# amazon-science/instruct-video-to-video

Measured on AMD Instinct MI355X. Metric: denoised video-frames/sec (16f@256x384, 50 DDIM steps), higher is better.
Workload: dtype fp16; 1 GPU; C2: 1 clip/step = VAE-encode + 50 DDIM steps (3-way CFG, text 7.5 / video 1.5) + VAE-decode, 16 frames @ 256x384, random-init full-width UNet+VAE; 5 independent clips in flight per GPU (stacked into every UNet launch, B = 3 x clips); frames=16, height=256, width=384, ddim_steps=50, clips_per_gpu=5, parallelism=clip-parallel x1, one all_gather, hip_graph=True, cfg_branch_streams=False, concurrent_clips=5, clip_mode=stacked, driver_mode=False, full=False

## Files before the change

### instruct-video-to-video_amd/csrc/attention.hip

```cpp
#include "common.h"
#include "gemm_dma.h"
#include <cstdlib>
#include <algorithm>

typedef unsigned int uint4v __attribute__((ext_vector_type(4)));

__device__ __forceinline__ unsigned pack2h(float a, float b) {
    auto h = __builtin_amdgcn_cvt_pkrtz(a, b);
    return __builtin_bit_cast(unsigned, h);
}

typedef float float2v __attribute__((ext_vector_type(2)));
typedef _Float16 half2v __attribute__((ext_vector_type(2)));
__device__ __forceinline__ float col_max(float v) {
    float a = v, b = v;
    asm volatile("s_nop 1\n\tv_permlane16_swap_b32 %0, %1\n\ts_nop 1" : "+v"(a), "+v"(b));
    a = b = fmaxf(a, b);
    asm volatile("s_nop 1\n\tv_permlane32_swap_b32 %0, %1\n\ts_nop 1" : "+v"(a), "+v"(b));
    return fmaxf(a, b);
}
__device__ __forceinline__ float col_sum(float v) {
    float a = v, b = v;
    asm volatile("s_nop 1\n\tv_permlane16_swap_b32 %0, %1\n\ts_nop 1" : "+v"(a), "+v"(b));
    a = b = a + b;
    asm volatile("s_nop 1\n\tv_permlane32_swap_b32 %0, %1\n\ts_nop 1" : "+v"(a), "+v"(b));
    return a + b;
}

#ifndef ATTN_REP_PREFETCH
#define ATTN_REP_PREFETCH 1
#endif
#ifndef ATTN_SINGLE_ST16
#define ATTN_SINGLE_ST16 1
#endif
template <int D, int NW, int KVT, int QB, bool FOLD = false, bool SINGLE = false, bool REP = false>
__global__ __launch_bounds__(NW * 64, (NW == 8 && D == 40) ? 4 : SINGLE ? 3 : (D == 80 && QB == 2) ? 2 : 1) void attn_kernel(insv2v_attention_desc p) {
    constexpr int NBUF = SINGLE ? 1 : 2;
    static_assert(!(SINGLE && FOLD), "the single-tile form is for the unfolded kernel");
    static_assert(!REP || SINGLE, "only the single-tile form keeps its tile across problems");
    constexpr int DP = (D + 31) / 32 * 32;
    constexpr int DTA = (D + 15) / 16;
    static_assert(!FOLD || DP > D, "FOLD needs a zero-padded contraction column");
    constexpr bool ONES = FOLD && (D % 16) != 0;
    constexpr int FKK = D / 32, FG = (D % 32) / 8, FE = D % 8;
    constexpr bool VDMA = FOLD && KVT == 64 && (D % 8) == 0 && (D % 16 == 0 || ONES);
    constexpr bool ST16 = SINGLE && !REP && ATTN_SINGLE_ST16 && (DTA % 2 == 0) && (D % 32 == 0);
    constexpr int NCBF = D / 16;
    constexpr bool VHALF = (D % 16) != 0;
    constexpr int VIMG = NCBF * KVT * 32 + (VHALF ? KVT * 16 : 0);
    constexpr int NPV = VIMG / 1024, NPVW = (NPV + NW - 1) / NW;
    constexpr int VT_LD = KVT + 4;
    constexpr int NKB = KVT / 32;
    constexpr bool KSWZ = DP == 64;
    constexpr int KLD = KSWZ ? DP : DP + 8;
    constexpr int DT = DP / 16;
    constexpr int KS = DP / 32;
    constexpr int NT = NW * 64;
    constexpr int KCH = DP / 8;
    constexpr int K_ITERS = (KVT * KCH + NT - 1) / NT;
    constexpr int VP = KVT / 2;
    constexpr int V_ITERS = (VP * KCH + NT - 1) / NT;
    extern __shared__ __attribute__((aligned(16))) char smem[];
    half_t* sK = (half_t*)smem;
    half_t* sVt = sK + NBUF * KVT * KLD;

    const int tid = threadIdx.x, lane = tid & 63, wid = tid >> 6;
    const int g = lane >> 4, qc = lane & 15;
    const int nqb = (p.seq_q + 16 * NW * QB - 1) / (16 * NW * QB), nhd = p.heads;
    const int lin = xcd_remap(blockIdx.x, gridDim.x);
    const int qblk = lin % nqb, head = (lin / nqb) % nhd;
    const int nrep = REP ? p.kv_inner : 1;
    const int z0 = (lin / (nqb * nhd)) * nrep;
    constexpr int d = D;
    const half_t* K = (const half_t*)p.k + (int64_t)(z0 / p.kv_inner) * p.kv_outer + (int64_t)(z0 % p.kv_inner) * p.kv_step + head * d;
    const half_t* V = (const half_t*)p.v + (int64_t)(z0 / p.kv_inner) * p.kv_outer + (int64_t)(z0 % p.kv_inner) * p.kv_step + head * d;

    int qrow[QB];
    half8 qf[QB][KS];
#pragma unroll
    for (int b = 0; b < QB; ++b) qrow[b] = (qblk * NW + wid) * (16 * QB) + b * 16 + qc;
    auto load_q = [&](int z) {
        const half_t* Q = (const half_t*)p.q + (int64_t)(z / p.q_inner) * p.q_outer + (int64_t)(z % p.q_inner) * p.q_step + head * d;
#pragma unroll
        for (int b = 0; b < QB; ++b) {
#pragma unroll
            for (int kk = 0; kk < KS; ++kk) {
                const int c = kk * 32 + g * 8;
                half8 v = {0, 0, 0, 0, 0, 0, 0, 0};
                if (qrow[b] < p.seq_q && c < d) v = *(const half8*)(Q + (int64_t)qrow[b] * p.q_rs + c);
                if (FOLD) {
                    const float c2q = p.scale * 1.4426950408889634f;
#pragma unroll
                    for (int e = 0; e < 8; ++e) v[e] = (half_t)((float)v[e] * c2q);
                }
                qf[b][kk] = v;
            }
        }
    };
    load_q(z0);
    const unsigned kone = (FOLD && g == FG) ? ((FE & 1) ? 0x3C000000u : 0x00003C00u) : 0u;

    uint4 rk[K_ITERS], rv[V_ITERS][2];
    const srd_t rK = make_srd(K), rVv = make_srd(V);
    constexpr int KROW_B = KLD * 2;
    constexpr bool KDMA = (KVT * KROW_B) % 1024 == 0;
    constexpr int NPK = KVT * KROW_B / 1024, NPKW = (NPK + NW - 1) / NW;
    static_assert(!VDMA || KDMA, "the V DMA path shares the K path's end-of-tile wait");
    int kd_key[KDMA ? NPKW : 1];
    unsigned kd_src[KDMA ? NPKW : 1];
    unsigned kd_off[KDMA ? NPKW : 1] = {};
    if (KDMA) {
#pragma unroll
        for (int i = 0; i < NPKW; ++i) {
            const int o = (wid + NW * i) * 1024 + lane * 16;
            const int key = o / KROW_B, slot = (o - key * KROW_B) >> 4;
            const int ch = KSWZ ? (slot ^ ((key >> 1) & 7)) : slot;
            kd_key[i] = (wid + NW * i < NPK && ch * 8 < d) ? key : (1 << 30);
            kd_src[i] = (unsigned)((key * (int)p.k_rs + ch * 8) * 2);
        }
    }
    int vd_key[VDMA ? NPVW : 1];
    unsigned vd_src[VDMA ? NPVW : 1];
    unsigned vd_off[VDMA ? NPVW : 1] = {};
    char* const sV = (char*)(sK + NBUF * KVT * KLD);
    if (VDMA) {
#pragma unroll
        for (int i = 0; i < NPVW; ++i) {
            const int pc = wid + NW * i;
            const bool full = pc < 2 * NCBF;
            const int key = full ? (pc & 1) * 32 + (lane >> 1) : lane;
            const int ch = full ? (pc >> 1) * 16 + (lane & 1) * 8 : NCBF * 16;
            vd_key[i] = pc < NPV ? key : (1 << 30);
            vd_src[i] = (unsigned)((key * (int)p.v_rs + ch) * 2);
        }
        if (tid < 4) ((unsigned*)(sV + 2 * VIMG))[tid] = tid == 0 ? 0x00003C00u : 0u;
    }
    auto load_vdma = [&](int t, int buf) {
        const int key0 = t * KVT;
#pragma unroll
        for (int i = 0; i < NPVW; ++i) {
            vd_off[i] = key0 + vd_key[i] < p.seq_k ? vd_src[i] : OOB_OFFSET;
            if (wid + NW * i < NPV)
                dma16(rVv, vd_off[i], key0 * (int)p.v_rs * 2, sV + buf * VIMG + (wid + NW * i) * 1024);
        }
    };
    auto load_k = [&](int t, int buf) {
        const int key0 = t * KVT;
        if (KDMA) {
            char* dst = (char*)(sK + buf * KVT * KLD) + wid * 1024;
#pragma unroll
            for (int i = 0; i < NPKW; ++i) {
                kd_off[i] = key0 + kd_key[i] < p.seq_k ? kd_src[i] : OOB_OFFSET;
                if (wid + NW * i < NPK)
                    dma16(rK, kd_off[i], key0 * (int)p.k_rs * 2, dst + i * NW * 1024);
            }
            return;
        }
#pragma unroll
        for (int i = 0; i < K_ITERS; ++i) {
            const int e = tid + NT * i;
            const int key = e / KCH, ch = e - key * KCH;
            const bool ok = e < KVT * KCH && key0 + key < p.seq_k && ch * 8 < d;
            const uint4v v = __builtin_amdgcn_raw_buffer_load_b128(rK, ok ? (unsigned)(((key0 + key) * (int)p.k_rs + ch * 8) * 2) : OOB_OFFSET, 0, 0);
            rk[i] = make_uint4(v[0], v[1], v[2], v[3]);
        }
    };
    auto load_v = [&](int t) {
        const int key0 = t * KVT;
#pragma unroll
        for (int i = 0; i < V_ITERS; ++i) {
            const int e = tid + NT * i;
            const int ch = e / VP, kp = e - ch * VP;
#pragma unroll
            for (int h = 0; h < 2; ++h) {
                const int key = key0 + 2 * kp + h;
                const bool ok = e < VP * KCH && key < p.seq_k && ch * 8 < d;
                const uint4v v = __builtin_amdgcn_raw_buffer_load_b128(rVv, ok ? (unsigned)((key * (int)p.v_rs + ch * 8) * 2) : OOB_OFFSET, 0, 0);
                rv[i][h] = make_uint4(v[0], v[1], v[2], v[3]);
            }
        }
    };
    auto load_tile = [&](int t, int buf) {
        if constexpr (VDMA) load_vdma(t, buf);
        else load_v(t);
        load_k(t, buf);
    };
    auto store_tile = [&](int buf) {
        half_t* k = sK + buf * KVT * KLD;
        half_t* vt = sVt + buf * DP * VT_LD;
#pragma unroll
        for (int i = 0; i < K_ITERS; ++i) {
            const int e = tid + NT * i;
            const int key = e / KCH, ch = e - key * KCH;
            const int pc = KSWZ ? (ch ^ ((key >> 1) & 7)) : ch;
            if (!KDMA && e < KVT * KCH) *(uint4*)(k + key * KLD + pc * 8) = rk[i];
        }
        if constexpr (VDMA) return;
#pragma unroll
        for (int i = 0; i < V_ITERS; ++i) {
            const int e = tid + NT * i;
            const int ch = e / VP, kp = e - ch * VP;
            if (e < VP * KCH) {
                const unsigned short* h0 = (const unsigned short*)&rv[i][0];
                const unsigned short* h1 = (const unsigned short*)&rv[i][1];
#pragma unroll
                for (int j = 0; j < 8; ++j) {
                    unsigned w = (unsigned)h0[j] | ((unsigned)h1[j] << 16);
                    if (ONES && j == D % 8 && ch == D / 8) w = 0x3C003C00u;
                    *(unsigned*)(vt + (ch * 8 + j) * VT_LD + 2 * kp) = w;
                }
            }
        }
    };

    floatx4 acc[QB][DT];
    float m_run[QB], l_run[QB];
    const float c2 = p.scale * 1.4426950408889634f;

    const unsigned sv_lds = (unsigned)(uintptr_t)(__attribute__((address_space(3))) char*)sV;
    const unsigned va_full = sv_lds + (g * 4 + (qc >> 2)) * 32 + (qc & 3) * 8;
    const bool va_const = (qc & 3) >= 2;
    const unsigned va_half0 = va_const ? sv_lds + 2 * VIMG + ((qc & 3) == 3 ? 8 : 0) : sv_lds + NCBF * KVT * 32 + (g * 4 + (qc >> 2)) * 16 + (qc & 3) * 8;
    const unsigned va_hstep_buf = va_const ? 0u : (unsigned)VIMG, va_hstep_kb = va_const ? 0u : 512u, va_hstep_hi = va_const ? 0u : 256u;

    const int ntiles = (p.seq_k + KVT - 1) / KVT;
    load_tile(0, 0);
    store_tile(0);
    if (KDMA) wait_vmcnt<0>();
    __syncthreads();

#pragma unroll 1
  for (int rep = 0; rep < nrep; ++rep) {
    const int z = z0 + rep;
#if !ATTN_REP_PREFETCH
    if (REP && rep > 0) load_q(z);
#endif
    half_t* O = (half_t*)p.o + (int64_t)(z / p.o_inner) * p.o_outer + (int64_t)(z % p.o_inner) * p.o_step + head * d;
#pragma unroll
    for (int b = 0; b < QB; ++b) {
        m_run[b] = FOLD ? 0.f : -1.0e30f;
        l_run[b] = 0.f;
#pragma unroll
        for (int i = 0; i < DT; ++i) acc[b][i] = (floatx4){0.f, 0.f, 0.f, 0.f};
    }
    for (int t = 0; t < ntiles; ++t) {
        const int cur = t & 1;
        const half_t* k = sK + cur * KVT * KLD;
        const half_t* vt = sVt + cur * DP * VT_LD;
        const int key0 = t * KVT;
        const bool ragged = key0 + KVT > p.seq_k;

        floatx4 s[QB][NKB][2];
#pragma unroll
        for (int kb = 0; kb < NKB; ++kb)
#pragma unroll
            for (int sub = 0; sub < 2; ++sub) {
#pragma unroll
                for (int b = 0; b < QB; ++b) s[b][kb][sub] = (floatx4){0.f, 0.f, 0.f, 0.f};
                const half_t* kr = k + (kb * 32 + sub * 16 + qc) * KLD;
                const int ksw = KSWZ ? ((qc >> 1) & 7) : 0;
#pragma unroll
                for (int kk = 0; kk < KS; ++kk) {
                    half8 kf = *(const half8*)(kr + (((kk * 4 + g) ^ ksw) * 8));
                    if (FOLD && kk == FKK) {
                        uint4v ku = __builtin_bit_cast(uint4v, kf);
                        ku[FE / 2] |= kone;
                        kf = __builtin_bit_cast(half8, ku);
                    }
#pragma unroll
                    for (int b = 0; b < QB; ++b)
                        s[b][kb][sub] = __builtin_amdgcn_mfma_f32_16x16x32_f16(kf, qf[b][kk], s[b][kb][sub], 0, 0, 0);
                }
            }
        if (t + 1 < ntiles) load_tile(t + 1, cur ^ 1);
#if ATTN_REP_PREFETCH
        if (REP && rep + 1 < nrep) load_q(z + 1);
#endif
        half8 pf[QB][NKB];
#pragma unroll
        for (int b = 0; b < QB; ++b) {
            if (ragged || p.causal) {
                const int kmax = p.causal ? min(p.seq_k - 1, qrow[b]) : p.seq_k - 1;
                const int rel = kmax - key0 - g * 4;
#pragma unroll
                for (int kb = 0; kb < NKB; ++kb)
#pragma unroll
                    for (int sub = 0; sub < 2; ++sub)
#pragma unroll
                        for (int r = 0; r < 4; ++r)
                            if (kb * 32 + sub * 16 + r > rel) s[b][kb][sub][r] = -1.0e30f;
            }
            if constexpr (FOLD) {
                float mx = s[b][0][0][0];
#pragma unroll
                for (int kb = 0; kb < NKB; ++kb)
#pragma unroll
                    for (int sub = 0; sub < 2; ++sub)
#pragma unroll
                        for (int r = 0; r < 4; ++r) mx = fmaxf(mx, s[b][kb][sub][r]);
                if (t == 0 || __builtin_amdgcn_ballot_w64(mx > 8.f) != 0) {
                    mx = col_max(mx);
                    const float want = m_run[b] + (t == 0 ? mx : fmaxf(mx, 0.f));
                    const float mnew = (float)(half_t)want;
                    const float shift = mnew - m_run[b];
                    m_run[b] = mnew;
                    if (t > 0) {
                        const float alpha = __builtin_amdgcn_exp2f(-shift);
                        if (!ONES) l_run[b] *= alpha;
#pragma unroll
                        for (int i = 0; i < DTA; ++i)
#pragma unroll
                            for (int r = 0; r < 4; ++r) acc[b][i][r] *= alpha;
                    }
#pragma unroll
                    for (int kb = 0; kb < NKB; ++kb)
#pragma unroll
                        for (int sub = 0; sub < 2; ++sub)
#pragma unroll
                            for (int r = 0; r < 4; ++r) s[b][kb][sub][r] -= shift;
                    if (g == FG) qf[b][FKK][FE] = (half_t)(-mnew);
                }
                const half2v ones = {(_Float16)1.f, (_Float16)1.f};
                float psum = 0.f;
#pragma unroll
                for (int kb = 0; kb < NKB; ++kb) {
                    uint4v pk;
#pragma unroll
                    for (int sub = 0; sub < 2; ++sub)
#pragma unroll
                        for (int h = 0; h < 2; ++h) {
                            const unsigned u = pack2h(__builtin_amdgcn_exp2f(s[b][kb][sub][2 * h]), __builtin_amdgcn_exp2f(s[b][kb][sub][2 * h + 1]));
                            if (!ONES) psum = __builtin_amdgcn_fdot2(__builtin_bit_cast(half2v, u), ones, psum, false);
                            pk[sub * 2 + h] = u;
                        }
                    pf[b][kb] = __builtin_bit_cast(half8, pk);
                }
                if (!ONES) l_run[b] += psum;
                continue;
            }
            float mx = m_run[b];
#pragma unroll
            for (int kb = 0; kb < NKB; ++kb)
#pragma unroll
                for (int sub = 0; sub < 2; ++sub)
#pragma unroll
                    for (int r = 0; r < 4; ++r) mx = fmaxf(mx, s[b][kb][sub][r]);
            mx = col_max(mx);
            if (__builtin_amdgcn_ballot_w64(mx > m_run[b]) != 0) {
                const float alpha = __builtin_amdgcn_exp2f((m_run[b] - mx) * c2);
                m_run[b] = mx;
                l_run[b] *= alpha;
#pragma unroll
                for (int i = 0; i < DTA; ++i)
#pragma unroll
                    for (int r = 0; r < 4; ++r) acc[b][i][r] *= alpha;
            }
            const float2v c2v = {c2, c2}, mcv = {-mx * c2, -mx * c2};
            const half2v ones = {(_Float16)1.f, (_Float16)1.f};
            float psum = 0.f;
#pragma unroll
            for (int kb = 0; kb < NKB; ++kb) {
                uint4v pk;
#pragma unroll
                for (int sub = 0; sub < 2; ++sub)
#pragma unroll
                    for (int h = 0; h < 2; ++h) {
                        float2v x = {s[b][kb][sub][2 * h], s[b][kb][sub][2 * h + 1]};
                        x = __builtin_elementwise_fma(x, c2v, mcv);
                        const unsigned u = pack2h(__builtin_amdgcn_exp2f(x[0]), __builtin_amdgcn_exp2f(x[1]));
                        psum = __builtin_amdgcn_fdot2(__builtin_bit_cast(half2v, u), ones, psum, false);
                        pk[sub * 2 + h] = u;
                    }
                pf[b][kb] = __builtin_bit_cast(half8, pk);
            }
            l_run[b] += psum;
        }

#pragma unroll
        for (int kb = 0; kb < NKB; ++kb) {
#pragma unroll
            for (int i = 0; i < DTA; ++i) {
                half4 lo, hi;
                if constexpr (VDMA) {
                    typedef __fp16 fp16x4 __attribute__((__vector_size__(4 * sizeof(__fp16))));
                    typedef __attribute__((address_space(3))) fp16x4* lds4_t;
                    if (i < NCBF) {
                        const unsigned a = va_full + cur * VIMG + i * (KVT * 32) + kb * 1024;
                        lo = __builtin_bit_cast(half4, __builtin_amdgcn_ds_read_tr16_b64_v4f16((lds4_t)(uintptr_t)a));
                        hi = __builtin_bit_cast(half4, __builtin_amdgcn_ds_read_tr16_b64_v4f16((lds4_t)(uintptr_t)(a + 512)));
                    } else {
                        const unsigned a = va_half0 + cur * va_hstep_buf + kb * va_hstep_kb;
                        lo = __builtin_bit_cast(half4, __builtin_amdgcn_ds_read_tr16_b64_v4f16((lds4_t)(uintptr_t)a));
                        hi = __builtin_bit_cast(half4, __builtin_amdgcn_ds_read_tr16_b64_v4f16((lds4_t)(uintptr_t)(a + va_hstep_hi)));
                    }
                } else {
                    const int vrow = ST16 ? (i >> 1) * 32 + 8 * (qc >> 2) + 4 * (i & 1) + (qc & 3) : i * 16 + qc;
                    const half_t* vr = vt + vrow * VT_LD + kb * 32 + g * 4;
                    lo = *(const half4*)vr;
                    hi = *(const half4*)(vr + 16);
                }
                const half8 vf = {lo[0], lo[1], lo[2], lo[3], hi[0], hi[1], hi[2], hi[3]};
#pragma unroll
                for (int b = 0; b < QB; ++b)
                    acc[b][i] = __builtin_amdgcn_mfma_f32_16x16x32_f16(vf, pf[b][kb], acc[b][i], 0, 0, 0);
            }
        }
        if (t + 1 < ntiles) store_tile(cur ^ 1);
        if (KDMA) {
#pragma unroll
            for (int i = 0; i < NPKW; ++i) asm volatile("" :: "v"(kd_off[i]));
            if (VDMA) {
#pragma unroll
                for (int i = 0; i < NPVW; ++i) asm volatile("" :: "v"(vd_off[i]));
            }
            wait_vmcnt<0>();
        }
        if (!REP) __syncthreads();
    }

#pragma unroll
    for (int b = 0; b < QB; ++b) {
        const float inv = 1.f / (ONES ? __shfl(acc[b][D / 16][D % 4], qc + 16 * ((D % 16) / 4), 64) : col_sum(l_run[b]));
        if (ST16) {
            if (qrow[b] < p.seq_q) {
                half_t* orow = O + (int64_t)qrow[b] * p.o_rs;
#pragma unroll
                for (int pp = 0; pp < DTA / 2; ++pp) {
                    const int c = pp * 32 + g * 8;
                    if (c < d) {
                        const floatx4 a0 = acc[b][2 * pp], a1 = acc[b][2 * pp + 1];
                        const half8 h = {(half_t)(a0[0] * inv), (half_t)(a0[1] * inv), (half_t)(a0[2] * inv), (half_t)(a0[3] * inv),
                                         (half_t)(a1[0] * inv), (half_t)(a1[1] * inv), (half_t)(a1[2] * inv), (half_t)(a1[3] * inv)};
                        *(half8*)(orow + c) = h;
                    }
                }
            }
            continue;
        }
        if (qrow[b] < p.seq_q) {
            half_t* orow = O + (int64_t)qrow[b] * p.o_rs;
#pragma unroll
            for (int i = 0; i < DTA; ++i) {
                const int c = i * 16 + g * 4;
                if (c < d) {
                    half4 h = {(half_t)(acc[b][i][0] * inv), (half_t)(acc[b][i][1] * inv), (half_t)(acc[b][i][2] * inv),
                               (half_t)(acc[b][i][3] * inv)};
                    *(half4*)(orow + c) = h;
                }
            }
        }
    }
  }
}


#ifndef ATTN_SHORT_MAXT
#define ATTN_SHORT_MAXT 512
#endif
template <int D, bool BIAS = false>
__global__ __launch_bounds__(BIAS ? ATTN_SHORT_MAXT : 1024) void attn_short_kernel(insv2v_attention_desc p) {
    constexpr int KS = (D + 31) / 32;
    constexpr int DT = (D + 15) / 16;
    constexpr int KCH = D / 8;
    constexpr int VT_LD = 20;
    constexpr int V_ITERS = (8 * KCH + 63) / 64;
    extern __shared__ __attribute__((aligned(16))) char smem[];
    const int lane = threadIdx.x & 63, head = __builtin_amdgcn_readfirstlane(threadIdx.x >> 6);
    const int g = lane >> 4, qc = lane & 15;
    half_t* vt = (half_t*)smem + head * (DT * 16 * VT_LD);
    const half8 z8 = {0, 0, 0, 0, 0, 0, 0, 0};
    half8 qb[KS], kb[KS], vb[V_ITERS][2];
    if (BIAS) {
#pragma unroll
        for (int kk = 0; kk < KS; ++kk) {
            const int c = kk * 32 + g * 8;
            const bool okq = c < D && qc < p.seq_q, okk = c < D && qc < p.seq_k;
            const half8 tq = *(const half8*)((const half_t*)p.q_bias + (okq ? (int64_t)qc * p.bias_rs + head * D + c : 0));
            const half8 tk = *(const half8*)((const half_t*)p.k_bias + (okk ? (int64_t)qc * p.bias_rs + head * D + c : 0));
            qb[kk] = okq ? tq : z8; kb[kk] = okk ? tk : z8;
        }
#pragma unroll
        for (int i = 0; i < V_ITERS; ++i) {
            const int e = lane + 64 * i;
            const int ch = e >> 3, kp = e & 7;
#pragma unroll
            for (int h = 0; h < 2; ++h) {
                const int key = 2 * kp + h;
                const bool okv = ch < KCH && key < p.seq_k;
                const half8 b = *(const half8*)((const half_t*)p.v_bias + (okv ? (int64_t)key * p.bias_rs + head * D + ch * 8 : 0));
                vb[i][h] = okv ? b : z8;
            }
        }
    }
#pragma unroll 1
  for (int z = blockIdx.x; z < p.batch; z += gridDim.x) {
    const half_t* Q = (const half_t*)p.q + (int64_t)(z / p.q_inner) * p.q_outer + (int64_t)(z % p.q_inner) * p.q_step + head * D;
    const half_t* K = (const half_t*)p.k + (int64_t)(z / p.kv_inner) * p.kv_outer + (int64_t)(z % p.kv_inner) * p.kv_step + head * D;
    const half_t* V = (const half_t*)p.v + (int64_t)(z / p.kv_inner) * p.kv_outer + (int64_t)(z % p.kv_inner) * p.kv_step + head * D;
    half_t* O = (half_t*)p.o + (int64_t)(z / p.o_inner) * p.o_outer + (int64_t)(z % p.o_inner) * p.o_step + head * D;

    const srd_t rV = make_srd(V);
    half8 qf[KS], kf[KS];
#pragma unroll
    for (int kk = 0; kk < KS; ++kk) {
        const int c = kk * 32 + g * 8;
        const bool okq = c < D && qc < p.seq_q, okk = c < D && qc < p.seq_k;
        half8 tq = *(const half8*)(Q + (okq ? (int64_t)qc * p.q_rs + c : 0));
        half8 tk = *(const half8*)(K + (okk ? (int64_t)qc * p.k_rs + c : 0));
        if (BIAS) {
            tq += qb[kk];
            tk += kb[kk];
        }
        qf[kk] = okq ? tq : z8; kf[kk] = okk ? tk : z8;
    }
    uint4 rv[V_ITERS][2];
#pragma unroll
    for (int i = 0; i < V_ITERS; ++i) {
        const int e = lane + 64 * i;
        const int ch = e >> 3, kp = e & 7;
#pragma unroll
        for (int h = 0; h < 2; ++h) {
            const int key = 2 * kp + h;
            const bool okv = ch < KCH && key < p.seq_k;
            uint4v t = __builtin_amdgcn_raw_buffer_load_b128(rV, okv ? (unsigned)((key * (int)p.v_rs + ch * 8) * 2) : OOB_OFFSET, 0, 0);
            if (BIAS) t = __builtin_bit_cast(uint4v, __builtin_bit_cast(half8, t) + vb[i][h]);
            rv[i][h] = make_uint4(t[0], t[1], t[2], t[3]);
        }
    }
    __builtin_amdgcn_sched_barrier(0);
    floatx4 s = {0.f, 0.f, 0.f, 0.f};
#pragma unroll
    for (int kk = 0; kk < KS; ++kk) s = __builtin_amdgcn_mfma_f32_16x16x32_f16(kf[kk], qf[kk], s, 0, 0, 0);
#pragma unroll
    for (int i = 0; i < V_ITERS; ++i) {
        const int e = lane + 64 * i;
        const int ch = e >> 3, kp = e & 7;
        if (ch < KCH) {
            const unsigned short* h0 = (const unsigned short*)&rv[i][0];
            const unsigned short* h1 = (const unsigned short*)&rv[i][1];
#pragma unroll
            for (int j = 0; j < 8; ++j) *(unsigned*)(vt + (ch * 8 + j) * VT_LD + 2 * kp) = (unsigned)h0[j] | ((unsigned)h1[j] << 16);
        }
    }
    const float c2 = p.scale * 1.4426950408889634f;
#pragma unroll
    for (int r = 0; r < 4; ++r)
        if (g * 4 + r >= p.seq_k) s[r] = -1.0e30f;
    float mx = fmaxf(fmaxf(s[0], s[1]), fmaxf(s[2], s[3]));
    mx = col_max(mx);
    const float mc = -mx * c2;
    float e[4], l = 0.f;
#pragma unroll
    for (int r = 0; r < 4; ++r) {
        e[r] = __builtin_amdgcn_exp2f(fmaf(s[r], c2, mc));
        l += e[r];
    }
    l = col_sum(l);
    const float inv = 1.f / l;
    const half4 pf = {(half_t)e[0], (half_t)e[1], (half_t)e[2], (half_t)e[3]};
    __builtin_amdgcn_wave_barrier();
    half_t* orow = O + (int64_t)qc * p.o_rs;
#pragma unroll
    for (int dt = 0; dt < DT; ++dt) {
        const half4 vf = *(const half4*)(vt + (dt * 16 + qc) * VT_LD + g * 4);
        floatx4 o = {0.f, 0.f, 0.f, 0.f};
        o = __builtin_amdgcn_mfma_f32_16x16x16f16(vf, pf, o, 0, 0, 0);
        const int c = dt * 16 + g * 4;
        if (c < D && qc < p.seq_q) {
            const half4 h = {(half_t)(o[0] * inv), (half_t)(o[1] * inv), (half_t)(o[2] * inv), (half_t)(o[3] * inv)};
            *(half4*)(orow + c) = h;
        }
    }
    __builtin_amdgcn_wave_barrier();
  }
}

template <int D>
static int launch_short(const insv2v_attention_desc& d, hipStream_t s) {
    constexpr int DT = (D + 15) / 16;
    const size_t lds = (size_t)d.heads * DT * 16 * 20 * sizeof(half_t);
    if (lds > 64 * 1024) return INSV2V_EUNSUPPORTED;
    if (d.q_bias && d.heads * 64 > ATTN_SHORT_MAXT) return INSV2V_EUNSUPPORTED;
    static const int wgs_per_cu = getenv("INSV2V_ATTN_SHORT_WGS") ? atoi(getenv("INSV2V_ATTN_SHORT_WGS")) : 2;
    static int cus = 0;
    if (!cus) {
        int dev = 0;
        hipDeviceProp_t prop;
        if (hipGetDevice(&dev) != hipSuccess || hipGetDeviceProperties(&prop, dev) != hipSuccess) return INSV2V_EINVAL;
        cus = prop.multiProcessorCount;
    }
    const int grid = (wgs_per_cu > 0 && d.q_bias) ? (int)std::min<int64_t>(d.batch, (int64_t)cus * wgs_per_cu) : d.batch;
    if (d.q_bias) hipLaunchKernelGGL((attn_short_kernel<D, true>), dim3(grid), dim3(d.heads * 64), lds, s, d);
    else hipLaunchKernelGGL((attn_short_kernel<D>), dim3(grid), dim3(d.heads * 64), lds, s, d);
    return launch_status();
}

static int dispatch_short(const insv2v_attention_desc& d, hipStream_t s) {
    switch (d.head_dim) {
        case 16: return launch_short<16>(d, s);
        case 32: return launch_short<32>(d, s);
        case 40: return launch_short<40>(d, s);
        case 64: return launch_short<64>(d, s);
        case 80: return launch_short<80>(d, s);
        case 128: return launch_short<128>(d, s);
        case 160: return launch_short<160>(d, s);
    }
    return INSV2V_EUNSUPPORTED;
}

template <int D, int NW, int QB, bool FOLD = false, int KVT_ = 0, bool SINGLE = false, bool REP = false>
static int launch_attn(const insv2v_attention_desc& d, hipStream_t s) {
    constexpr int DP = (D + 31) / 32 * 32;
    constexpr int KVT = KVT_ ? KVT_ : (NW >= 4 ? 64 : 32);
    constexpr size_t lds = (size_t)(SINGLE ? 1 : 2) * (KVT * (DP + 8) + DP * (KVT + 4)) * sizeof(half_t);
    if constexpr (!FOLD && !SINGLE && (D == 40 || D == 80) && NW >= 4) {
        static const int fold = getenv("INSV2V_ATTN_FOLD") ? atoi(getenv("INSV2V_ATTN_FOLD")) : 1;
        if (fold) return launch_attn<D, NW, QB, true>(d, s);
    }
    if (SINGLE && d.seq_k > KVT) return INSV2V_EUNSUPPORTED;
    static bool attr_set = false;
    if (!attr_set) {
        hipError_t e = hipFuncSetAttribute((const void*)attn_kernel<D, NW, KVT, QB, FOLD, SINGLE, REP>,
                                           hipFuncAttributeMaxDynamicSharedMemorySize, (int)lds);
        if (e != hipSuccess) return (int)e;
        attr_set = true;
    }
    constexpr int rows = 16 * NW * QB;
    if (REP && (d.kv_inner <= 1 || d.kv_step != 0 || d.batch % d.kv_inner)) return INSV2V_EUNSUPPORTED;
    const int64_t nwg = (int64_t)((d.seq_q + rows - 1) / rows) * d.heads * (REP ? d.batch / d.kv_inner : d.batch);
    if (nwg > 0x7fffffff) return INSV2V_EUNSUPPORTED;
    hipLaunchKernelGGL((attn_kernel<D, NW, KVT, QB, FOLD, SINGLE, REP>), dim3((unsigned)nwg), dim3(NW * 64), lds, s, d);
    return launch_status();
}

template <int NW, int QB>
static int dispatch_dp(const insv2v_attention_desc& d, hipStream_t s) {
    switch (d.head_dim) {
        case 16: return launch_attn<16, NW, QB>(d, s);
        case 32: return launch_attn<32, NW, QB>(d, s);
        case 40: return launch_attn<40, NW, QB>(d, s);
        case 64: return launch_attn<64, NW, QB>(d, s);
        case 80: return launch_attn<80, NW, QB>(d, s);
        case 128: return launch_attn<128, NW, QB>(d, s);
        case 160: return launch_attn<160, NW, QB>(d, s);
    }
    return INSV2V_EUNSUPPORTED;
}

extern "C" int insv2v_attention(const insv2v_attention_desc* dp, insv2v_stream_t stream) {
    if (!one_device()) return INSV2V_EINVAL;
    if (!dp) return INSV2V_EINVAL;
    insv2v_attention_desc d = *dp;
    if (!d.q || !d.k || !d.v || !d.o) return INSV2V_EINVAL;
    if (d.head_dim <= 0 || (d.head_dim & 7) || d.head_dim > 160) return INSV2V_EINVAL;
    if (d.seq_q <= 0 || d.seq_k <= 0 || d.batch <= 0 || d.heads <= 0) return INSV2V_EINVAL;
    if ((d.q_rs & 7) || (d.k_rs & 7) || (d.v_rs & 7) || (d.o_rs & 3)) return INSV2V_EINVAL;
    if (d.q_inner <= 0) d.q_inner = 1;
    if (d.kv_inner <= 0) d.kv_inner = 1;
    if (d.o_inner <= 0) d.o_inner = 1;
    hipStream_t s = as_stream(stream);
    static const int short_on = getenv("INSV2V_ATTN_SHORT") ? atoi(getenv("INSV2V_ATTN_SHORT")) : 1;
    const bool biased = d.q_bias || d.k_bias || d.v_bias;
    if (biased && (!d.q_bias || !d.k_bias || !d.v_bias || (d.bias_rs & 7) || ((uintptr_t)d.q_bias & 15) || ((uintptr_t)d.k_bias & 15) || ((uintptr_t)d.v_bias & 15)))
        return INSV2V_EINVAL;
    if ((short_on || biased) && d.seq_q <= 16 && d.seq_k <= 16 && !d.causal && d.heads <= 16) {
        const int rc = dispatch_short(d, s);
        if (rc != INSV2V_EUNSUPPORTED || biased) return rc;
    }
    if (biased) return INSV2V_EUNSUPPORTED;
    static const int single_on = getenv("INSV2V_ATTN_SINGLE") ? atoi(getenv("INSV2V_ATTN_SINGLE")) : 1;
    const bool o16 = !(d.o_rs & 7) && !((uintptr_t)d.o & 15) && !(d.o_outer & 7) && !(d.o_step & 7);
    if (single_on && o16 && d.head_dim == 160 && !d.causal && d.seq_q > 64 && d.seq_q <= 96 && d.seq_k <= 96) {
        static const int rep_on = getenv("INSV2V_ATTN_REP") ? atoi(getenv("INSV2V_ATTN_REP")) : 1;
        if (rep_on && d.kv_inner > 1 && d.kv_step == 0 && d.batch % d.kv_inner == 0) return launch_attn<160, 6, 1, false, 96, true, true>(d, s);
        return launch_attn<160, 6, 1, false, 96, true>(d, s);
    }
    if (d.seq_q <= 16) return dispatch_dp<1, 1>(d, s);
    if (d.seq_q <= 32) return dispatch_dp<2, 1>(d, s);
    if (d.seq_q >= 512 && d.seq_q % 256 == 0 && d.head_dim <= 96) return dispatch_dp<8, 2>(d, s);
    if (d.seq_q >= 128 && d.head_dim <= 96) return dispatch_dp<4, 2>(d, s);
    return dispatch_dp<4, 1>(d, s);
}
```

Before: 16.90 frames/s.

## Replace per-tile max check in folded attention with lazy sum-based rescale and redo fallback

In the FOLD attention path, the per-tile row-max reduction and ballot are dropped after the first tile. Rescaling now happens only when the running denominator crosses a threshold, with the new offset derived from the exponent of the sum. If the sum risks fp16 or float overflow, the whole block is flagged and the tile loop is rerun in the fully checked mode. This removes a max reduction from every tile, at the cost of more code and a possible full recompute for blocks with large logits.

```diff
diff --git a/instruct-video-to-video_amd/csrc/attention.hip b/instruct-video-to-video_amd/csrc/attention.hip
--- a/instruct-video-to-video_amd/csrc/attention.hip
+++ b/instruct-video-to-video_amd/csrc/attention.hip
@@ -2,6 +2,7 @@
 #include "gemm_dma.h"
 #include <cstdlib>
 #include <algorithm>
+#include <type_traits>
 
 typedef unsigned int uint4v __attribute__((ext_vector_type(4)));
 
@@ -27,6 +28,9 @@
     return a + b;
 }
 
+#ifdef ATTN_REDO_COUNT
+__device__ unsigned long long attn_redo_count;
+#endif
 #ifndef ATTN_REP_PREFETCH
 #define ATTN_REP_PREFETCH 1
 #endif
@@ -223,6 +227,10 @@
     const unsigned va_half0 = va_const ? sv_lds + 2 * VIMG + ((qc & 3) == 3 ? 8 : 0) : sv_lds + NCBF * KVT * 32 + (g * 4 + (qc >> 2)) * 16 + (qc & 3) * 8;
     const unsigned va_hstep_buf = va_const ? 0u : (unsigned)VIMG, va_hstep_kb = va_const ? 0u : 512u, va_hstep_hi = va_const ? 0u : 256u;
 
+    constexpr int LG = (D % 16) / 4;
+    constexpr unsigned long long LMASK = ONES ? 0xFFFFull << (16 * LG) : ~0ull;
+    constexpr float LTHR = ONES ? 256.f : 64.f;
+    int redo = 0;
     const int ntiles = (p.seq_k + KVT - 1) / KVT;
     load_tile(0, 0);
     store_tile(0);
@@ -243,6 +251,8 @@
 #pragma unroll
         for (int i = 0; i < DT; ++i) acc[b][i] = (floatx4){0.f, 0.f, 0.f, 0.f};
     }
+    auto run_tiles = [&](auto checked_tag) __attribute__((always_inline)) {
+    constexpr bool CHECKED = decltype(checked_tag)::value;
     for (int t = 0; t < ntiles; ++t) {
         const int cur = t & 1;
         const half_t* k = sK + cur * KVT * KLD;
@@ -291,6 +301,7 @@
                             if (kb * 32 + sub * 16 + r > rel) s[b][kb][sub][r] = -1.0e30f;
             }
             if constexpr (FOLD) {
+              if (CHECKED || t == 0) {
                 float mx = s[b][0][0][0];
 #pragma unroll
                 for (int kb = 0; kb < NKB; ++kb)
@@ -320,6 +331,37 @@
                             for (int r = 0; r < 4; ++r) s[b][kb][sub][r] -= shift;
                     if (g == FG) qf[b][FKK][FE] = (half_t)(-mnew);
                 }
+              } else {
+                const float lpart = ONES ? acc[b][D / 16][D % 4] : l_run[b];
+                if ((__builtin_amdgcn_ballot_w64(!(lpart <= LTHR)) & LMASK) != 0) {
+                    const float l = ONES ? __shfl(lpart, qc + 16 * LG, 64) : col_sum(lpart);
+                    const bool ok = l < 32768.f;
+                    if (__builtin_amdgcn_ballot_w64(!ok) != 0) redo = 1;
+                    const float ls = ok ? l : 1.f;
+                    const float fl = (float)(__builtin_amdgcn_frexp_expf(ls) - 1);
+                    float mnew = (float)(half_t)floorf(m_run[b] + fl);
+                    float shift = mnew - m_run[b];
+                    float alpha = __builtin_amdgcn_exp2f(-shift);
+                    if (ls * alpha >= 2.f) {
+                        mnew = (float)(half_t)(mnew + 1.f);
+                        shift = mnew - m_run[b];
+                        alpha = __builtin_amdgcn_exp2f(-shift);
+                    }
+                    m_run[b] = mnew;
+                    if (!ONES) l_run[b] *= alpha;
+#pragma unroll
+                    for (int i = 0; i < DTA; ++i)
+#pragma unroll
+                        for (int r = 0; r < 4; ++r) acc[b][i][r] *= alpha;
+#pragma unroll
+                    for (int kb = 0; kb < NKB; ++kb)
+#pragma unroll
+                        for (int sub = 0; sub < 2; ++sub)
+#pragma unroll
+                            for (int r = 0; r < 4; ++r) s[b][kb][sub][r] -= shift;
+                    if (g == FG) qf[b][FKK][FE] = (half_t)(-mnew);
+                }
+              }
                 const half2v ones = {(_Float16)1.f, (_Float16)1.f};
                 float psum = 0.f;
 #pragma unroll
@@ -417,6 +459,35 @@
         }
         if (!REP) __syncthreads();
     }
+    };
+    if constexpr (FOLD) {
+        run_tiles(std::false_type{});
+#pragma unroll
+        for (int b = 0; b < QB; ++b) {
+            const float lpart = ONES ? acc[b][D / 16][D % 4] : l_run[b];
+            if ((__builtin_amdgcn_ballot_w64(!(lpart < (ONES ? 32768.f : 8192.f))) & LMASK) != 0) redo = 1;
+        }
+        if (__syncthreads_or(redo)) {
+#ifdef ATTN_REDO_COUNT
+            if (tid == 0) atomicAdd(&attn_redo_count, 1ull);
+#endif
+#pragma unroll
+            for (int b = 0; b < QB; ++b) {
+                m_run[b] = 0.f;
+                l_run[b] = 0.f;
+#pragma unroll
+                for (int i = 0; i < DT; ++i) acc[b][i] = (floatx4){0.f, 0.f, 0.f, 0.f};
+                if (g == FG) qf[b][FKK][FE] = (half_t)0.f;
+            }
+            load_tile(0, 0);
+            store_tile(0);
+            if (KDMA) wait_vmcnt<0>();
+            __syncthreads();
+            run_tiles(std::true_type{});
+        }
+    } else {
+        run_tiles(std::true_type{});
+    }
 
 #pragma unroll
     for (int b = 0; b < QB; ++b) {
@@ -681,3 +752,12 @@
     if (d.seq_q >= 128 && d.head_dim <= 96) return dispatch_dp<4, 2>(d, s);
     return dispatch_dp<4, 1>(d, s);
 }
+
+#ifdef ATTN_REDO_COUNT
+extern "C" long long insv2v_attention_redo_count(int reset) {
+    unsigned long long v = 0, z = 0;
+    if (hipDeviceSynchronize() != hipSuccess || hipMemcpyFromSymbol(&v, HIP_SYMBOL(attn_redo_count), sizeof(v)) != hipSuccess) return -1;
+    if (reset && hipMemcpyToSymbol(HIP_SYMBOL(attn_redo_count), &z, sizeof(z)) != hipSuccess) return -1;
+    return (long long)v;
+}
+#endif
```

Result: no change. 16.89 frames/s (-0.1%).
